# sundy-li/strawboat

Measured on AMD Instinct MI355X. Metric: encode+decode GB/s (uncompressed Arrow bytes) per GPU; 1/2/4/8-GPU scaling, higher is better.
Workload: dtype f64 bit patterns (integer/bit work, no arithmetic); 1 GPU; C2: 512 x 1M-row nullable Float64 columns per GPU, 64Ki-row pages, codec adaptive, inputs resident in HBM; columns_per_gpu=512, rows_per_column=1000000, page_rows=65536, parallelism=pages of independent columns sharded across 1 GPU(s)

## Files before the change

strawboat_amd/csrc/sb_aggregate.h:

```cpp
#pragma once

namespace sb {

struct AggAcc {
    uint64_t cnt = 0, nans = 0, kmin = ~0ull, kmax = 0, s0 = 0, s1 = 0;
};
__device__ __forceinline__ bool agg_is_float(uint32_t kind) { return kind == FK_F32 || kind == FK_F64; }
__device__ __forceinline__ double agg_dbl(uint64_t b) { return __longlong_as_double((long long)b); }
__device__ __forceinline__ uint64_t agg_bits(double v) { return (uint64_t)__double_as_longlong(v); }
__device__ __forceinline__ uint64_t agg_sext(uint64_t raw, uint32_t w) {
    const uint32_t sh = 64 - 8 * w;
    return (uint64_t)((int64_t)(raw << sh) >> sh);
}
__device__ __forceinline__ uint64_t agg_key(uint32_t kind, uint32_t w, uint64_t raw) {
    if (kind == FK_UNSIGNED) return raw;
    if (kind == FK_SIGNED) return agg_sext(raw, w) ^ (1ull << 63);
    if (kind == FK_F32) {
        const uint32_t b = (uint32_t)raw;
        return (b >> 31) ? (uint32_t)~b : (b | 0x80000000u);
    }
    return (raw >> 63) ? ~raw : (raw | (1ull << 63));
}
__device__ __forceinline__ uint64_t agg_unkey(uint32_t kind, uint32_t w, uint64_t key) {
    if (kind == FK_UNSIGNED) return key;
// ... 198 lines not shown
            agg_span(k, acc, kind, w, lo, hi, [&](uint64_t r) { return (uint64_t)s_a[sidx((int)(r - lo))]; });
            break;
        }
        default:
            return;
    }
    acc = agg_wg_reduce(acc, agg_is_float(kind), s_red);
    if (threadIdx.x == 0) agg_store(al.parts + al.tile_base + t.first_tile + tt.tile, acc);
}

__global__ void __launch_bounds__(WG) k_agg(DecodeArgs a, AggLaunch al) {
    __shared__ uint32_t s_a[SIDX_WORDS];
    __shared__ uint32_t s_w[4];
    __shared__ uint64_t s_red[AGG_RED_WORDS];
    const uint32_t count = a.job_counts[2];
    for (uint32_t ti = blockIdx.x; ti < count; ti += gridDim.x) {
        agg_tile(a, al, ti, s_a, s_w, s_red);
        __syncthreads();
    }
}

struct RleAggregate {
    using Rec = uint64_t;
    uint64_t* s_rec;
    AggSink k;
    AggAcc* acc;
    uint32_t kind, w;
    __device__ __forceinline__ uint32_t rec_bytes() const { return 4 + w; }
    __device__ __forceinline__ uint64_t load(const uint8_t* v, bool in) const { return in ? flt_load(v, w) : 0ull; }
    __device__ __forceinline__ void rows(uint64_t tile_lo, uint64_t lo, uint64_t hi, uint32_t A, const uint32_t* s_flag) const {
        agg_span(k, *acc, kind, w, lo, hi, [&](uint64_t r) { return s_rec[A + s_flag[sidx((int)(r - tile_lo))]]; });
    }
};

__global__ void __launch_bounds__(WG) k_agg_rle(DecodeArgs a, AggLaunch al) {
    __shared__ __attribute__((aligned(16))) uint32_t s_flag[SIDX_WORDS];
    __shared__ uint64_t s_vals[RLE_CHUNK];
    __shared__ uint32_t s_w[4];
    __shared__ uint64_t s_w64[4];
    __shared__ uint64_t s_red[AGG_RED_WORDS];
    if (a.job_counts[4] == 0) return;
    const uint32_t p = blockIdx.x;
    const PageDesc d = a.descs[p];
    const PageTask t = a.tasks[p];
    const ColDesc c = a.cols[t.col];
    if (!rle_by_page(c, d)) return;
// ... 148 lines not shown
```

strawboat_amd/csrc/sb_aggregate_grouped.h:

```cpp
#pragma once

namespace sb {

typedef __attribute__((address_space(3))) uint64_t* l64p;
constexpr uint32_t GF_SEL = 0, GF_CNT = 1, GF_NANS = 2, GF_KMIN = 3, GF_KMAX = 4, GF_SUM = 5;
constexpr uint32_t GRP_TREE_IDS = 4;
constexpr uint32_t GRP_LDS_WORDS =(GF_SUM + WG / 64) * GRP_MAX_GROUPS;
template <uint32_t S = GRP_MAX_GROUPS>
__device__ __forceinline__ uint64_t* grp_field(uint64_t* s_g, uint32_t f) { return s_g + f * S; }
__device__ __forceinline__ void grp_lds_add(uint64_t* p, uint64_t v) {
    (void)__hip_atomic_fetch_add((l64p)p, v, __ATOMIC_RELAXED, __HIP_MEMORY_SCOPE_WORKGROUP);
}

struct GrpSink {
    const uint32_t* sel;
    const uint8_t* def_bits;
    uint64_t out_row;
    const uint8_t* ids;
    uint32_t idw, G;
    uint64_t* s_g;
    bool all_null;
};
__device__ __forceinline__ uint32_t grp_id(const uint8_t* ids, uint32_t w, uint64_t c) {
    return w == 1 ? (uint32_t)ldu8(ids + c) : w == 2 ? (uint32_t)ldu16(ids + 2 * c) : ldu32(ids + 4 * c);
// ... 199 lines not shown
    }
    if (!agg_any_selected(g.sel, t.out_row + lo, t.out_row + hi)) return;
    grp_table_clear(s_g, gc.n_groups);
    const GrpSink k{g.sel, d.def_bits, t.out_row, gc.ids, gc.idw, gc.n_groups, s_g, false};
    uint64_t oor = 0;
    if (!grp_tile_rows(a, d, t, c, k, oor, kind, tt.page, tt.tile, lo, hi, s_a, s_w)) return;
    grp_store(gl, tt.col, gl.tile_base + t.first_tile + tt.tile, gc.n_groups, agg_is_float(kind), s_g, oor, s_w64);
}

__global__ void __launch_bounds__(WG) k_grp(DecodeArgs a, GrpLaunch gl) {
    __shared__ uint32_t s_a[SIDX_WORDS];
    __shared__ uint32_t s_w[4];
    __shared__ uint64_t s_w64[4];
    __shared__ uint64_t s_g[GRP_LDS_WORDS];
    const uint32_t count = a.job_counts[2];
    for (uint32_t ti = blockIdx.x; ti < count; ti += gridDim.x) {
        grp_tile(a, gl, ti, s_a, s_w, s_g, s_w64);
        __syncthreads();
    }
}

struct RleGrouped {
    using Rec = uint64_t;
    uint64_t* s_rec;
    GrpSink k;
    uint64_t* oor;
    uint32_t kind, w;
    __device__ __forceinline__ uint32_t rec_bytes() const { return 4 + w; }
    __device__ __forceinline__ uint64_t load(const uint8_t* v, bool in) const { return in ? flt_load(v, w) : 0ull; }
    __device__ __forceinline__ void rows(uint64_t tile_lo, uint64_t lo, uint64_t hi, uint32_t A, const uint32_t* s_flag) const {
        grp_span<true>(k, *oor, kind, w, lo, hi, [&](uint64_t r, uint64_t& raw) { return raw = s_rec[A + s_flag[sidx((int)(r - tile_lo))]], true; });
    }
};

__global__ void __launch_bounds__(WG) k_grp_rle(DecodeArgs a, GrpLaunch gl) {
    __shared__ __attribute__((aligned(16))) uint32_t s_flag[SIDX_WORDS];
    __shared__ uint64_t s_vals[RLE_CHUNK];
    __shared__ uint32_t s_w[4];
    __shared__ uint64_t s_w64[4];
    __shared__ uint64_t s_g[GRP_LDS_WORDS];
    if (a.job_counts[4] == 0) return;
    const uint32_t p = blockIdx.x;
    const PageDesc d = a.descs[p];
    const PageTask t = a.tasks[p];
    const ColDesc c = a.cols[t.col];
    if (!rle_by_page(c, d)) return;
// ... 161 lines not shown
```

strawboat_amd/csrc/sb_aggregate_grouped_large.h:

```cpp
#pragma once

namespace sb {

constexpr uint32_t GRPL_LDS_WORDS = (GF_SUM + WG / 64) * GRPL_MAX_GROUPS;
constexpr uint32_t GRPL_FINISH_GROUPS = 256;

__device__ __forceinline__ bool grpl_tile(const DecodeArgs& a, const GrpLaunch& gl, uint32_t col, const ColDesc& c, const AggCol& g, const GrpCol& gc,
                                          uint32_t page, uint32_t tile, bool& live, uint64_t& oor, uint32_t* s_a, uint32_t* s_w, uint64_t* s_g) {
    const PageDesc d = a.descs[page];
    if (!d.ok) return false;
    const PageTask t = a.tasks[page];
    const uint64_t lo = (uint64_t)tile * TILE_ROWS;
    if (lo >= t.num_values) return false;
    const uint64_t hi = min(t.num_values, lo + TILE_ROWS);
    if (d.codec == SB_CODEC_FREQ) {
        if (threadIdx.x == 0 && tile == 0) {
            gst64(gl.flags + gl.slots + gl.n_cols + col, 1);
            if (gl.replayed) raise(a.status, SB_ERR_NYI, page, 411);
            else atomicOr(&a.status->kinds, KIND_REPLAY | KIND_FILTER_FREQ);
        }
        return false;
    }
    if (rle_by_page(c, d)) return false;
    if (!agg_any_selected(g.sel, t.out_row + lo, t.out_row + hi)) return false;
// ... 23 lines not shown
    const AggCol g = gl.acols[col];
    if (slot < g.tile_slot0 || slot - g.tile_slot0 >= g.tile_slots) return;
    if (!(g.ops & AGG_VALUE_OPS)) return;
    const ColDesc c = a.cols[col];
    if (!c.n_pages) return;
    const GrpCol gc = gl.gcols[col];
    const PageTask last = a.tasks[c.first_page + c.n_pages - 1];
    const uint64_t t0 = a.tasks[c.first_page].first_tile;
    const uint64_t t1 = (uint64_t)last.first_tile + (last.num_values + TILE_ROWS - 1) / TILE_ROWS;
    const uint64_t j0 = (slot - g.tile_slot0) * GRPL_CHUNK_TILES;
    const uint64_t j1 = min(t1 - t0, j0 + GRPL_CHUNK_TILES);
    bool live = false;
    uint64_t oor = 0;
    for (uint64_t j = j0; j < j1; j++) {
        const uint32_t gt = (uint32_t)(t0 + j);
        const uint32_t page = grpl_page_of(a.tasks, c.first_page, c.n_pages, gt);
        (void)grpl_tile(a, gl, col, c, g, gc, page, gt - a.tasks[page].first_tile, live, oor, s_a, s_w, s_g);
    }
    if (live) grp_store<GRPL_MAX_GROUPS>(gl, col, slot, gc.n_groups, agg_is_float(g.kind), s_g, oor, s_w64);
}

struct RleGroupedLarge {
    using Rec = uint64_t;
    uint64_t* s_rec;
    GrpSink k;
    uint64_t* oor;
    uint32_t kind, w;
    __device__ __forceinline__ uint32_t rec_bytes() const { return 4 + w; }
    __device__ __forceinline__ uint64_t load(const uint8_t* v, bool in) const { return in ? flt_load(v, w) : 0ull; }
    __device__ __forceinline__ void rows(uint64_t tile_lo, uint64_t lo, uint64_t hi, uint32_t A, const uint32_t* s_flag) const {
        grp_span<true, GRPL_MAX_GROUPS>(k, *oor, kind, w, lo, hi,
                                        [&](uint64_t r, uint64_t& raw) { return raw = s_rec[A + s_flag[sidx((int)(r - tile_lo))]], true; });
    }
};

__global__ void __launch_bounds__(WG) k_grpl_rle(DecodeArgs a, GrpLaunch gl) {
    __shared__ __attribute__((aligned(16))) uint32_t s_flag[SIDX_WORDS];
    __shared__ uint64_t s_vals[RLE_CHUNK];
    __shared__ uint32_t s_w[4];
    __shared__ uint64_t s_w64[4];
    __shared__ uint64_t s_g[GRPL_LDS_WORDS];
    if (a.job_counts[4] == 0) return;
    const uint32_t p = blockIdx.x;
    const PageDesc d = a.descs[p];
    const PageTask t = a.tasks[p];
    const ColDesc c = a.cols[t.col];
// ... 175 lines not shown
```

strawboat_amd/csrc/sb_aggregate_weighted.h:

```cpp
#pragma once

namespace sb {

constexpr uint32_t WF_SEL = 0, WF_CNT = 1, WF_NANS = 2, WF_SUM = 3;
constexpr uint32_t WGT_FIELDS = WF_SUM + WG / 64;
constexpr uint32_t WGT_LDS_WORDS = WGT_FIELDS * GRPL_MAX_GROUPS;

__device__ __forceinline__ uint64_t* wgt_field(uint64_t* s_g, uint32_t f) { return s_g + f * GRPL_MAX_GROUPS; }

__device__ __forceinline__ void wgt_table_clear(uint64_t* s_g, uint32_t G) {
    for (uint32_t i = threadIdx.x; i < G; i += WG) {
#pragma unroll
        for (uint32_t f = 0; f < WGT_FIELDS; f++) wgt_field(s_g, f)[i] = 0ull;
    }
    __syncthreads();
}

__device__ __forceinline__ uint64_t wgt_ext(uint32_t kind, uint32_t w, uint64_t raw) { return kind == FK_SIGNED ? agg_sext(raw, w) : raw; }
__device__ __forceinline__ double wgt_dbl(uint32_t kind, uint32_t w, uint64_t raw) {
    return kind == FK_F32 ? (double)__uint_as_float((uint32_t)raw) : kind == FK_F64 ? agg_dbl(raw) : kind == FK_SIGNED ? (double)(int64_t)agg_sext(raw, w) : (double)raw;
}

template <bool VAL, class V>
__device__ __forceinline__ void wgt_span(const GrpSink& k, const WgtCol& wc, uint64_t& oor, uint32_t kind, uint32_t w, uint64_t lo, uint64_t hi, V value_of) {
// ... 201 lines not shown
    if (slot < g.tile_slot0 || slot - g.tile_slot0 >= g.tile_slots) return;
    if (!(g.ops & AGG_VALUE_OPS)) return;
    const ColDesc c = a.cols[col];
    if (!c.n_pages) return;
    const GrpCol gc = gl.gcols[col];
    const WgtCol wc = wl.wcols[col];
    const PageTask last = a.tasks[c.first_page + c.n_pages - 1];
    const uint64_t t0 = a.tasks[c.first_page].first_tile;
    const uint64_t t1 = (uint64_t)last.first_tile + (last.num_values + TILE_ROWS - 1) / TILE_ROWS;
    const uint64_t j0 = (slot - g.tile_slot0) * GRPL_CHUNK_TILES;
    const uint64_t j1 = min(t1 - t0, j0 + GRPL_CHUNK_TILES);
    bool live = false;
    uint64_t oor = 0;
    for (uint64_t j = j0; j < j1; j++) {
        const uint32_t gt = (uint32_t)(t0 + j);
        const uint32_t page = grpl_page_of(a.tasks, c.first_page, c.n_pages, gt);
        wgt_tile(a, gl, col, c, g, gc, wc, page, gt - a.tasks[page].first_tile, live, oor, s_a, s_w, s_g);
    }
    if (live) wgt_store(gl, col, slot, gc.n_groups, wc.flt, s_g, oor, s_w64);
}

struct RleWeighted {
    using Rec = uint64_t;
    uint64_t* s_rec;
    GrpSink k;
    WgtCol wc;
    uint64_t* oor;
    uint32_t kind, w;
    __device__ __forceinline__ uint32_t rec_bytes() const { return 4 + w; }
    __device__ __forceinline__ uint64_t load(const uint8_t* v, bool in) const { return in ? flt_load(v, w) : 0ull; }
    __device__ __forceinline__ void rows(uint64_t tile_lo, uint64_t lo, uint64_t hi, uint32_t A, const uint32_t* s_flag) const {
        wgt_span<true>(k, wc, *oor, kind, w, lo, hi, [&](uint64_t r, uint64_t& raw) { return raw = s_rec[A + s_flag[sidx((int)(r - tile_lo))]], true; });
    }
};

__global__ void __launch_bounds__(WG) k_wgt_rle(DecodeArgs a, WgtLaunch wl) {
    __shared__ __attribute__((aligned(16))) uint32_t s_flag[SIDX_WORDS];
    __shared__ uint64_t s_vals[RLE_CHUNK];
    __shared__ uint32_t s_w[4];
    __shared__ uint64_t s_w64[4];
    __shared__ uint64_t s_g[WGT_LDS_WORDS];
    if (a.job_counts[4] == 0) return;
    const GrpLaunch& gl = wl.gl;
    const uint32_t p = blockIdx.x;
    const PageDesc d = a.descs[p];
    const PageTask t = a.tasks[p];
// ... 184 lines not shown
```

strawboat_amd/csrc/sb_decode.hip:

```cpp
#include "sb_host.h"
#include "sb_zstd.h"
#include "sb_zstd_blocks.h"
#include "sb_lz4.h"
#include "sb_lz4_big.h"
#include "sb_lz4_giant.h"

namespace sb {

__device__ __forceinline__ bool is_basic(uint32_t c) { return c <= 3; }
__device__ __forceinline__ bool is_binary(int32_t t) { return t == SB_TYPE_BINARY || t == SB_TYPE_LARGE_BINARY; }
__device__ __forceinline__ uint32_t ballot_half(uint64_t m) { return (threadIdx.x & 32) ? (uint32_t)(m >> 32) : (uint32_t)m; }

__device__ __forceinline__ void push_job(InflateJob* q, uint32_t* cnt, const uint8_t* src, uint32_t csize,
                                         uint8_t* dst, uint32_t out_len, uint32_t codec, uint32_t page);
__device__ __forceinline__ void push_job_if(bool pred, InflateJob* q, uint32_t* cnt, const uint8_t* src, uint32_t csize, uint8_t* dst,
                                            uint32_t out_len, uint32_t codec, uint32_t page) {
    const uint64_t m = __ballot(pred);
    if (!m) return;
    const uint32_t rank = __builtin_amdgcn_mbcnt_hi((uint32_t)(m >> 32), __builtin_amdgcn_mbcnt_lo((uint32_t)m, 0));
    uint32_t base = 0;
    if (pred && rank == 0) base = __hip_atomic_fetch_add(cnt, (uint32_t)__popcll(m), __ATOMIC_RELAXED, __HIP_MEMORY_SCOPE_AGENT);
    base = (uint32_t)__builtin_amdgcn_readlane((int)base, __builtin_ctzll(m));
    if (pred) {
        InflateJob j;
// ... 2482 lines not shown
                              const uint64_t* sums ) {
    const uint32_t REC = p.rec_bytes();
    const int tid = threadIdx.x;
    const uint64_t N = t.num_values;
    const uint8_t* body = d.body;
    const uint8_t* page_end = c.pages + t.in_off + t.length;
    const uint32_t max_runs = (uint32_t)((uint64_t)(page_end - body) / REC);
    uint32_t ncnt[RLE_RPT];
    typename P::Rec nrec[RLE_RPT];
    auto fetch = [&](uint32_t base) {
#pragma unroll
        for (int j = 0; j < RLE_RPT; j++) {
            const uint32_t k = base + (uint32_t)tid * RLE_RPT + j;
            const bool in = k < max_runs;
            const uint8_t* r = body + (uint64_t)(in ? k : 0) * REC;
            ncnt[j] = in ? ldu32(r) : 0;
            nrec[j] = p.load(r + 4, in);
        }
    };
    const RlePart pt = rle_part(max_runs, part, parts);
    if (pt.none) return;
    uint64_t carry = 0;
    for (uint32_t q = 0; q < part; q++) carry += sums[q];
    if (max_runs) fetch(pt.b0);
    for (uint64_t base64 = pt.b0; carry < N && base64 < pt.b1; base64 += RLE_CHUNK) {
        const uint32_t base = (uint32_t)base64;
        if (base64 >= max_runs) {
            if (tid == 0) raise(st, SB_ERR_IO, page, 200);
            return;
        }
        uint32_t cnt[RLE_RPT];
#pragma unroll
        for (int j = 0; j < RLE_RPT; j++) {
            cnt[j] = ncnt[j];
            p.s_rec[tid * RLE_RPT + j] = nrec[j];
        }
        if (base + RLE_CHUNK < max_runs) fetch(base + RLE_CHUNK);
        uint64_t loc[RLE_RPT], run = 0;
#pragma unroll
        for (int j = 0; j < RLE_RPT; j++) {
            run += cnt[j];
            loc[j] = run;
        }
        const uint64_t incl = wave_incl_scan64(run);
        __syncthreads();
        if ((tid & 63) == 63) s_w64[tid >> 6] = incl;
        __syncthreads();
        uint64_t pre = carry + incl - run;
        const int w = tid >> 6;
        if (w > 0) pre += s_w64[0];
        if (w > 1) pre += s_w64[1];
        if (w > 2) pre += s_w64[2];
        const uint64_t chunk_total = s_w64[0] + s_w64[1] + s_w64[2] + s_w64[3];
        uint64_t start[RLE_RPT];
#pragma unroll
        for (int j = 0; j < RLE_RPT; j++) start[j] = pre + (j ? loc[j - 1] : 0);
        const uint64_t S0 = carry, S1 = min(N, carry + chunk_total);
#pragma unroll
        for (int j = 0; j < RLE_RPT; j++)
            if (start[j] < N && start[j] + cnt[j] > N) raise(st, SB_ERR_OUT_OF_SPEC, page, 202);
        for (uint64_t tile_lo = S0 / TILE_ROWS * TILE_ROWS; tile_lo < S1; tile_lo += TILE_ROWS) {
            const uint64_t lo = max(S0, tile_lo), hi = min(S1, tile_lo + TILE_ROWS);
            static_assert(SIDX_WORDS % 4 == 0, "16-byte clears");
            for (int i = tid; i < SIDX_WORDS / 4; i += WG) ((u32x4*)s_flag)[i] = u32x4{0, 0, 0, 0};
            uint32_t le = 0;
#pragma unroll
            for (int j = 0; j < RLE_RPT; j++) le += (base + (uint32_t)tid * RLE_RPT + j < max_runs && start[j] <= lo) ? 1u : 0u;
            __syncthreads();
#pragma unroll
            for (int j = 0; j < RLE_RPT; j++)
                if (base + (uint32_t)tid * RLE_RPT + j < max_runs && start[j] > lo && start[j] < hi)
                    atomicAdd(&s_flag[sidx((int)(start[j] - tile_lo))], 1u);
            uint32_t v = le;
#pragma unroll
            for (int dlt = 32; dlt > 0; dlt >>= 1) v += __shfl_down(v, dlt, 64);
            if ((tid & 63) == 0) s_w[tid >> 6] = v;
            __syncthreads();
            const uint32_t A = s_w[0] + s_w[1] + s_w[2] + s_w[3] - 1;
            __syncthreads();
            tile_incl_scan(s_flag, s_w);
            p.rows(tile_lo, lo, hi, A, s_flag);
            __syncthreads();
        }
        carry += chunk_total;
        if (chunk_total == 0 && base + RLE_CHUNK >= max_runs && carry < N) {
            if (tid == 0) raise(st, SB_ERR_IO, page, 200);
            return;
        }
    }
}

template <int W>
struct RleExpand {
    using Rec = Val<W>;
    Val<W>* s_rec;
    uint8_t* dst;
    __device__ __forceinline__ uint32_t rec_bytes() const { return 4 + W; }
    __device__ __forceinline__ Val<W> load(const uint8_t* v, bool in) const { return in ? ld_val<W>(v) : Val<W>{}; }
    __device__ __forceinline__ void rows(uint64_t tile_lo, uint64_t lo, uint64_t hi, uint32_t A, const uint32_t* s_flag) const {
        const uint32_t off = (uint32_t)(lo - tile_lo);
        emit_rows<W>(dst + lo * W, (uint32_t)(hi - lo), [&](uint32_t i) { return s_rec[A + s_flag[sidx((int)(off + i))]]; });
    }
};
template <int W>
__device__ __forceinline__ void expand_rle_page(const ColDesc& c, const PageTask& t, const PageDesc& d, uint32_t* s_flag, uint8_t* s_vals,
                                                uint32_t* s_w, uint64_t* s_w64, Status* st, uint32_t page, uint32_t part, uint32_t parts,
                                                const uint64_t* sums) {
    rle_page_walk(RleExpand<W>{(Val<W>*)s_vals, c.values + t.out_row * W}, c, t, d, s_flag, s_w, s_w64, st, page, part, parts, sums);
}

__device__ void page_copy_bits(uint8_t* dst_bm, uint64_t dst_bit0, const uint8_t* src, uint64_t N, bool aligned) {
    constexpr int U = 8;
    const uint32_t nwords = (uint32_t)((N + 31) / 32);
    for (uint32_t g0 = threadIdx.x; g0 < nwords; g0 += WG * U) {
        uint32_t v[U];
#pragma unroll
        for (int u = 0; u < U; u++) {
// ... 386 lines not shown
```

strawboat_amd/csrc/sb_filter.h:

```cpp
#pragma once

namespace sb {

constexpr uint32_t FILTER_DICT_BITS = 8192;

struct FilterCmp {
    uint64_t lit;
    uint32_t kind, mask, w;
};
__device__ __forceinline__ FilterCmp filter_cmp(const FilterCol& f, uint32_t w) { return FilterCmp{f.lit, f.kind, f.mask, w}; }
__device__ __forceinline__ uint64_t flt_load(const uint8_t* p, uint32_t w) {
    switch (w) {
        case 1:
            return ldu8(p);
        case 2:
            return ldu16(p);
        case 4:
            return ldu32(p);
        default:
            return ldu64(p);
    }
}
__device__ __forceinline__ bool flt_eval(const FilterCmp& k, uint64_t raw) {
    uint32_t rel;
// ... 141 lines not shown
            U32Stream vs{d.body, (const uint32_t*)(a.scratch + t.aux_off), d.codec, 0, t.num_values};
            u32_tile_to_lds(vs, tt.tile, rows, s_a, s_w);
            filter_span(k, lo, hi, [&](uint64_t r) { return flt_eval(cmp, s_a[sidx((int)(r - lo))]); });
            break;
        }
        default:
            break;
    }
}

__global__ void __launch_bounds__(WG) k_filter(DecodeArgs a, const FilterCol* fcols) {
    __shared__ uint32_t s_a[SIDX_WORDS];
    __shared__ uint32_t s_w[4];
    __shared__ uint32_t s_tab[FILTER_DICT_BITS / 32];
    const uint32_t count = a.job_counts[2];
    for (uint32_t ti = blockIdx.x; ti < count; ti += gridDim.x) {
        filter_tile(a, fcols, ti, s_a, s_w, s_tab);
        __syncthreads();
    }
}

struct RleFilter {
    using Rec = uint8_t;
    uint8_t* s_rec;
    FilterSink k;
    FilterCmp cmp;
    __device__ __forceinline__ uint32_t rec_bytes() const { return 4 + cmp.w; }
    __device__ __forceinline__ uint8_t load(const uint8_t* v, bool in) const { return in && flt_eval(cmp, flt_load(v, cmp.w)); }
    __device__ __forceinline__ void rows(uint64_t tile_lo, uint64_t lo, uint64_t hi, uint32_t A, const uint32_t* s_flag) const {
        filter_span(k, lo, hi, [&](uint64_t r) { return s_rec[A + s_flag[sidx((int)(r - tile_lo))]] != 0; });
    }
};

__global__ void __launch_bounds__(WG) k_filter_rle(DecodeArgs a, const FilterCol* fcols) {
    __shared__ __attribute__((aligned(16))) uint32_t s_flag[SIDX_WORDS];
    __shared__ uint8_t s_pred[RLE_CHUNK];
    __shared__ uint32_t s_w[4];
    __shared__ uint64_t s_w64[4];
    if (a.job_counts[4] == 0) return;
    const uint32_t p = blockIdx.x;
    const PageDesc d = a.descs[p];
    const PageTask t = a.tasks[p];
    const ColDesc c = a.cols[t.col];
    if (!rle_by_page(c, d)) return;
    const FilterCol f = fcols[t.col];
    if (f.op >= SB_PRED_IS_NULL) return;
// ... 108 lines not shown
```

strawboat_amd/csrc/sb_filter_in.h:

```cpp
#pragma once

namespace sb {

struct InEval {
    const uint64_t* keys;
    uint32_t n, steps, negate, kind, w;
};
__device__ __forceinline__ bool in_member(const uint64_t* keys, uint32_t n, uint32_t steps, uint64_t x) {
    uint32_t pos = 0;
    for (uint32_t s = steps; s-- > 0;) {
        const uint32_t p = pos + (1u << s);
        const uint64_t k = keys[min(p, n) - 1];
        pos = (p <= n && k < x) ? p : pos;
    }
    return n != 0 && pos < n && keys[min(pos, n - 1)] == x;
}
__device__ __forceinline__ bool in_eval(const InEval& k, uint64_t raw) {
    return in_member(k.keys, k.n, k.steps, in_key(k.kind, k.w, raw)) != (k.negate != 0);
}
__device__ __forceinline__ void in_stage(const InCol& ic, uint64_t* s_keys) {
    const uint32_t n = min(ic.n, IN_MAX_VALUES);
    for (uint32_t i = threadIdx.x; i < n; i += WG) s_keys[i] = ic.keys[i];
}
__device__ __forceinline__ InEval in_eval_of(const FilterCol& f, const InCol& ic, const uint64_t* s_keys, uint32_t w) {
// ... 71 lines not shown
            filter_span(k, lo, hi, [&](uint64_t r) { return in_eval(ev, s_a[sidx((int)(r - lo))]); });
            break;
        }
        default:
            break;
    }
}

__global__ void __launch_bounds__(WG) k_filter_in(DecodeArgs a, const FilterCol* fcols, const InCol* icols) {
    __shared__ uint32_t s_a[SIDX_WORDS];
    __shared__ uint32_t s_w[4];
    __shared__ uint32_t s_tab[FILTER_DICT_BITS / 32];
    __shared__ uint64_t s_keys[IN_MAX_VALUES];
    const uint32_t count = a.job_counts[2];
    uint32_t staged = 0xFFFFFFFFu;
    for (uint32_t ti = blockIdx.x; ti < count; ti += gridDim.x) {
        filter_in_tile(a, fcols, icols, ti, s_a, s_w, s_tab, s_keys, &staged);
        __syncthreads();
    }
}

struct RleFilterIn {
    using Rec = uint8_t;
    uint8_t* s_rec;
    FilterSink k;
    InEval ev;
    __device__ __forceinline__ uint32_t rec_bytes() const { return 4 + ev.w; }
    __device__ __forceinline__ uint8_t load(const uint8_t* v, bool in) const { return in && in_eval(ev, flt_load(v, ev.w)); }
    __device__ __forceinline__ void rows(uint64_t tile_lo, uint64_t lo, uint64_t hi, uint32_t A, const uint32_t* s_flag) const {
        filter_span(k, lo, hi, [&](uint64_t r) { return s_rec[A + s_flag[sidx((int)(r - tile_lo))]] != 0; });
    }
};

__global__ void __launch_bounds__(WG) k_filter_in_rle(DecodeArgs a, const FilterCol* fcols, const InCol* icols) {
    __shared__ __attribute__((aligned(16))) uint32_t s_flag[SIDX_WORDS];
    __shared__ uint8_t s_pred[RLE_CHUNK];
    __shared__ uint32_t s_w[4];
    __shared__ uint64_t s_w64[4];
    __shared__ uint64_t s_keys[IN_MAX_VALUES];
    if (a.job_counts[4] == 0) return;
    const uint32_t p = blockIdx.x;
    const PageDesc d = a.descs[p];
    const PageTask t = a.tasks[p];
    const ColDesc c = a.cols[t.col];
    if (!rle_by_page(c, d)) return;
    const FilterCol f = fcols[t.col];
// ... 173 lines not shown
```

strawboat_amd/csrc/sb_key_buckets.h:

```cpp
#pragma once

namespace sb {

constexpr uint32_t BUCK_NAN = 0xFFFFu;
constexpr uint32_t BUCK_BAD = 0xFFFEu;
static_assert(BUCK_MAX_BOUNDS + 1 <= KEY_MAX_KEYS && BUCK_MAX_BOUNDS < BUCK_BAD, "a bucket code fits 16 bits beside the markers");

struct BuckFind {
    const uint64_t* keys;
    const uint32_t* bid;
    uint64_t nan_lo, nan_hi;
    uint32_t n, steps, kind, w, rc, nan_id;
};
template <bool FLT>
__device__ __forceinline__ uint32_t buck_code(const BuckFind& f, uint64_t raw) {
    const uint64_t x = in_key(f.kind, f.w, raw);
    uint32_t pos = key_lower_bound(f.keys, f.n, f.steps, x);
    if (!f.rc && pos < f.n && f.keys[pos] == x) pos++;
    if (FLT && (x < f.nan_lo || x > f.nan_hi)) pos = BUCK_NAN;
    return pos;
}
__device__ __forceinline__ uint32_t buck_id(const BuckFind& f, uint32_t code) {
    return code <= f.n ? f.bid[code] : code == BUCK_NAN ? f.nan_id : LOOK_NONE;
}
// ... 155 lines not shown
    if (flt) key_buckets_rows<true>(a, tt, d, t, c, b, f, lo, rows, s_a, s_w, s_pos);
    else key_buckets_rows<false>(a, tt, d, t, c, b, f, lo, rows, s_a, s_w, s_pos);
    buck_store(b, flt, bl.st + tt.col, s_cnt);
}

__global__ void __launch_bounds__(WG) k_key_buckets(DecodeArgs a, BuckLaunch bl) {
    __shared__ uint32_t s_a[SIDX_WORDS];
    __shared__ uint32_t s_w[4];
    __shared__ unsigned long long s_cnt[3];
    __shared__ uint16_t s_pos[FILTER_DICT_BITS];
    __shared__ uint64_t s_keys[KEY_MAX_KEYS];
    __shared__ uint32_t s_bid[KEY_MAX_KEYS];
    const uint32_t count = a.job_counts[2];
    uint32_t staged = 0xFFFFFFFFu;
    for (uint32_t ti = blockIdx.x; ti < count; ti += gridDim.x) {
        key_buckets_tile(a, bl, ti, s_a, s_w, s_pos, s_keys, s_bid, s_cnt, &staged);
        __syncthreads();
    }
}

template <bool FLT>
struct RleKeyBuckets {
    using Rec = uint32_t;
    uint32_t* s_rec;
    BuckSink* b;
    BuckFind f;
    __device__ __forceinline__ uint32_t rec_bytes() const { return 4 + f.w; }
    __device__ __forceinline__ uint32_t load(const uint8_t* v, bool in) const {
        if (!in) return FLT ? BUCK_BAD : LOOK_NONE;
        const uint32_t code = buck_code<FLT>(f, flt_load(v, f.w));
        return FLT ? code : buck_id(f, code);
    }
    __device__ __forceinline__ void rows(uint64_t tile_lo, uint64_t lo, uint64_t hi, uint32_t A, const uint32_t* s_flag) const {
        if (FLT) buck_span_f(*b, f, lo, hi, [&](uint64_t r) { return s_rec[A + s_flag[sidx((int)(r - tile_lo))]]; });
        else look_span(b->k, lo, hi, [&](uint64_t r) { return s_rec[A + s_flag[sidx((int)(r - tile_lo))]]; });
    }
};

__global__ void __launch_bounds__(WG) k_key_buckets_rle(DecodeArgs a, BuckLaunch bl) {
    __shared__ __attribute__((aligned(16))) uint32_t s_flag[SIDX_WORDS];
    __shared__ uint32_t s_run[RLE_CHUNK];
    __shared__ uint32_t s_w[4];
    __shared__ uint64_t s_w64[4];
    __shared__ unsigned long long s_cnt[3];
    __shared__ uint64_t s_keys[KEY_MAX_KEYS];
    __shared__ uint32_t s_bid[KEY_MAX_KEYS];
// ... 99 lines not shown
```

strawboat_amd/csrc/sb_key_ids.h:

```cpp
#pragma once

namespace sb {

constexpr uint32_t KEY_SET_SLOTS = 2048;
static_assert(KEY_SET_SLOTS >= KEY_MAX_KEYS + 2 * WG && (KEY_SET_SLOTS & (KEY_SET_SLOTS - 1)) == 0, "never full; a power of two");

__device__ __forceinline__ uint32_t key_hash(uint64_t key) { return (uint32_t)((key * 0x9E3779B97F4A7C15ull) >> 40); }
__device__ __forceinline__ uint32_t key_over(const KeyState* st) {
    return __hip_atomic_load(&st->overflow, __ATOMIC_RELAXED, __HIP_MEMORY_SCOPE_AGENT);
}

struct KeySink {
    const uint32_t* sel;
    const uint8_t* def_bits;
    uint64_t out_row;
    uint64_t* set;
    KeyState* st;
    uint64_t* tab;
    uint32_t mask, max_keys;
    uint64_t cnt = 0;
    uint32_t zero = 0;
};
__device__ __forceinline__ KeySink key_sink(const KeyLaunch& kl, uint32_t col, uint64_t* set, const uint32_t* sel, const uint8_t* def_bits, uint64_t out_row) {
    const KeyCol kc = kl.kcols[col];
// ... 158 lines not shown
        }
        default:
            return;
    }
    key_store(s, s_w64);
}

__global__ void __launch_bounds__(WG) k_key_collect(DecodeArgs a, KeyLaunch kl) {
    __shared__ uint32_t s_a[SIDX_WORDS];
    __shared__ uint32_t s_w[4];
    __shared__ uint64_t s_w64[4];
    __shared__ uint32_t s_tab[FILTER_DICT_BITS / 32];
    __shared__ uint64_t s_set[KEY_SET_SLOTS];
    const uint32_t count = a.job_counts[2];
    uint32_t owner = 0xFFFFFFFFu;
    for (uint32_t ti = blockIdx.x; ti < count; ti += gridDim.x) {
        key_collect_tile(a, kl, ti, s_a, s_w, s_tab, s_set, s_w64, &owner);
        __syncthreads();
    }
}

struct RleKeyCollect {
    using Rec = uint64_t;
    uint64_t* s_rec;
    KeySink* k;
    uint32_t kind, w;
    __device__ __forceinline__ uint32_t rec_bytes() const { return 4 + w; }
    __device__ __forceinline__ uint64_t load(const uint8_t* v, bool in) const { return in ? in_key(kind, w, flt_load(v, w)) : 0ull; }
    __device__ __forceinline__ void rows(uint64_t tile_lo, uint64_t lo, uint64_t hi, uint32_t A, const uint32_t* s_flag) const {
        key_span(*k, lo, hi, [&](uint64_t r) { return s_rec[A + s_flag[sidx((int)(r - tile_lo))]]; });
    }
};

__global__ void __launch_bounds__(WG) k_key_collect_rle(DecodeArgs a, KeyLaunch kl) {
    __shared__ __attribute__((aligned(16))) uint32_t s_flag[SIDX_WORDS];
    __shared__ uint64_t s_vals[RLE_CHUNK];
    __shared__ uint32_t s_w[4];
    __shared__ uint64_t s_w64[4];
    __shared__ uint64_t s_set[KEY_SET_SLOTS];
    if (a.job_counts[4] == 0) return;
    const uint32_t p = blockIdx.x;
    const PageDesc d = a.descs[p];
    const PageTask t = a.tasks[p];
    const ColDesc c = a.cols[t.col];
    if (!rle_by_page(c, d)) return;
    const AggCol g = kl.acols[t.col];
// ... 193 lines not shown
            key_id_span(k, lo, hi, [&](uint64_t r) { return key_find(f, (uint64_t)s_a[sidx((int)(r - lo))]); });
            break;
        }
        default:
            break;
    }
}

__global__ void __launch_bounds__(WG) k_key_assign(DecodeArgs a, KeyLaunch kl) {
    __shared__ uint32_t s_a[SIDX_WORDS];
    __shared__ uint32_t s_w[4];
    __shared__ uint16_t s_ids[FILTER_DICT_BITS];
    __shared__ uint64_t s_keys[KEY_MAX_KEYS];
    const uint32_t count = a.job_counts[2];
    uint32_t staged = 0xFFFFFFFFu;
    for (uint32_t ti = blockIdx.x; ti < count; ti += gridDim.x) {
        key_assign_tile(a, kl, ti, s_a, s_w, s_ids, s_keys, &staged);
        __syncthreads();
    }
}

struct RleKeyAssign {
    using Rec = uint32_t;
    uint32_t* s_rec;
    KeyIdSink k;
    KeyFind f;
    __device__ __forceinline__ uint32_t rec_bytes() const { return 4 + f.w; }
    __device__ __forceinline__ uint32_t load(const uint8_t* v, bool in) const { return in ? key_find(f, flt_load(v, f.w)) : 0u; }
    __device__ __forceinline__ void rows(uint64_t tile_lo, uint64_t lo, uint64_t hi, uint32_t A, const uint32_t* s_flag) const {
        key_id_span(k, lo, hi, [&](uint64_t r) { return s_rec[A + s_flag[sidx((int)(r - tile_lo))]]; });
    }
};

__global__ void __launch_bounds__(WG) k_key_assign_rle(DecodeArgs a, KeyLaunch kl) {
    __shared__ __attribute__((aligned(16))) uint32_t s_flag[SIDX_WORDS];
    __shared__ uint32_t s_run[RLE_CHUNK];
    __shared__ uint32_t s_w[4];
    __shared__ uint64_t s_w64[4];
    __shared__ uint64_t s_keys[KEY_MAX_KEYS];
    if (a.job_counts[4] == 0) return;
    const uint32_t p = blockIdx.x;
    const PageDesc d = a.descs[p];
    const PageTask t = a.tasks[p];
    const ColDesc c = a.cols[t.col];
    if (!rle_by_page(c, d)) return;
    if (kl.st[t.col].overflow) return;
// ... 71 lines not shown
```

strawboat_amd/csrc/sb_key_lookup.h:

```cpp
#pragma once

namespace sb {

constexpr uint32_t LOOK_NONE = 0xFFFFFFFFu;
constexpr uint32_t LOOK_NOPOS = 0xFFFFu;
static_assert(KEY_MAX_KEYS <= LOOK_NOPOS, "a sorted position fits 16 bits beside the marker");

struct LookSink {
    const uint32_t* sel;
    const uint8_t* def_bits;
    uint64_t out_row;
    uint8_t* ids;
    uint32_t idw;
    uint32_t live = 0, hit = 0;
};
template <class F>
__device__ __forceinline__ void look_span(LookSink& k, uint64_t lo, uint64_t hi, F id_of) {
    for (uint64_t base = lo; base < hi; base += WG) {
        const uint64_t r = base + threadIdx.x, c = k.out_row + r;
        const bool in = r < hi;
        bool on = in;
        if (on && k.sel) on = (gld32(k.sel + (c >> 5)) >> (uint32_t)(c & 31)) & 1u;
        if (on && k.def_bits) on = (ldu8(k.def_bits + (r >> 3)) >> (uint32_t)(r & 7)) & 1u;
        const uint32_t id = on ? id_of(r) : LOOK_NONE;
// ... 125 lines not shown
        default:
            return;
    }
    look_store(k, ll.st + tt.col, s_cnt);
}

__global__ void __launch_bounds__(WG) k_key_lookup(DecodeArgs a, LookLaunch ll) {
    __shared__ uint32_t s_a[SIDX_WORDS];
    __shared__ uint32_t s_w[4];
    __shared__ unsigned long long s_cnt[2];
    __shared__ uint16_t s_pos[FILTER_DICT_BITS];
    __shared__ uint64_t s_keys[KEY_MAX_KEYS];
    __shared__ uint32_t s_kid[KEY_MAX_KEYS];
    const uint32_t count = a.job_counts[2];
    uint32_t staged = 0xFFFFFFFFu;
    for (uint32_t ti = blockIdx.x; ti < count; ti += gridDim.x) {
        key_lookup_tile(a, ll, ti, s_a, s_w, s_pos, s_keys, s_kid, s_cnt, &staged);
        __syncthreads();
    }
}

struct RleKeyLookup {
    using Rec = uint32_t;
    uint32_t* s_rec;
    LookSink* k;
    LookFind f;
    __device__ __forceinline__ uint32_t rec_bytes() const { return 4 + f.w; }
    __device__ __forceinline__ uint32_t load(const uint8_t* v, bool in) const { return in ? look_find(f, flt_load(v, f.w)) : LOOK_NONE; }
    __device__ __forceinline__ void rows(uint64_t tile_lo, uint64_t lo, uint64_t hi, uint32_t A, const uint32_t* s_flag) const {
        look_span(*k, lo, hi, [&](uint64_t r) { return s_rec[A + s_flag[sidx((int)(r - tile_lo))]]; });
    }
};

__global__ void __launch_bounds__(WG) k_key_lookup_rle(DecodeArgs a, LookLaunch ll) {
    __shared__ __attribute__((aligned(16))) uint32_t s_flag[SIDX_WORDS];
    __shared__ uint32_t s_run[RLE_CHUNK];
    __shared__ uint32_t s_w[4];
    __shared__ uint64_t s_w64[4];
    __shared__ unsigned long long s_cnt[2];
    __shared__ uint64_t s_keys[KEY_MAX_KEYS];
    __shared__ uint32_t s_kid[KEY_MAX_KEYS];
    if (a.job_counts[4] == 0) return;
    const uint32_t p = blockIdx.x;
    const PageDesc d = a.descs[p];
    const PageTask t = a.tasks[p];
    const ColDesc c = a.cols[t.col];
// ... 208 lines not shown
```

strawboat_amd/csrc/sb_read_sel.h:

```cpp
#pragma once

namespace sb {

__device__ __forceinline__ uint64_t sel_rank_at(const SelCol& s, uint64_t c) {
    const uint64_t g = c >> 5;
    const uint32_t b = (uint32_t)(c & 31);
    uint64_t r = gld64(s.rank + g);
    if (b) r += (uint64_t)__popc(gld32(s.sel + g) & ((1u << b) - 1));
    return r;
}

__device__ __forceinline__ void sel_store(uint8_t* p, uint64_t v, uint32_t w) {
    switch (w) {
        case 1:
            *(gptr)p = (uint8_t)v;
            break;
        case 2: {
            const uint16_t x = (uint16_t)v;
            __builtin_memcpy((gptr)p, &x, 2);
            break;
        }
        case 4:
            stu32(p, (uint32_t)v);
            break;
// ... 125 lines not shown
            U32Stream vs{d.body, (const uint32_t*)(a.scratch + t.aux_off), d.codec, 0, t.num_values};
            u32_tile_to_lds(vs, tt.tile, rows, s_a, s_w);
            sel_span(k, lo, hi, [&](uint64_t r) { return (uint64_t)s_a[sidx((int)(r - lo))]; });
            break;
        }
        default:
            break;
    }
}

__global__ void __launch_bounds__(WG) k_rsel(DecodeArgs a, const SelCol* scols) {
    __shared__ uint32_t s_a[SIDX_WORDS];
    __shared__ uint32_t s_w[4];
    __shared__ uint32_t s_strip[WG];
    const uint32_t count = a.job_counts[2];
    for (uint32_t ti = blockIdx.x; ti < count; ti += gridDim.x) {
        rsel_tile(a, scols, ti, s_a, s_w, s_strip);
        __syncthreads();
    }
}

struct RleSelect {
    using Rec = uint64_t;
    uint64_t* s_rec;
    SelSink k;
    __device__ __forceinline__ uint32_t rec_bytes() const { return 4 + k.s.w; }
    __device__ __forceinline__ uint64_t load(const uint8_t* v, bool in) const { return in ? flt_load(v, k.s.w) : 0ull; }
    __device__ __forceinline__ void rows(uint64_t tile_lo, uint64_t lo, uint64_t hi, uint32_t A, const uint32_t* s_flag) const {
        if (sel_rank_at(k.s, k.out_row + lo) == sel_rank_at(k.s, k.out_row + hi)) return;
        sel_span(k, lo, hi, [&](uint64_t r) { return s_rec[A + s_flag[sidx((int)(r - tile_lo))]]; });
    }
};

__global__ void __launch_bounds__(WG) k_rsel_rle(DecodeArgs a, const SelCol* scols) {
    __shared__ __attribute__((aligned(16))) uint32_t s_flag[SIDX_WORDS];
    __shared__ uint64_t s_vals[RLE_CHUNK];
    __shared__ uint32_t s_w[4];
    __shared__ uint64_t s_w64[4];
    __shared__ uint32_t s_strip[WG];
    if (a.job_counts[4] == 0) return;
    const uint32_t p = blockIdx.x;
    const PageDesc d = a.descs[p];
    const PageTask t = a.tasks[p];
    const ColDesc c = a.cols[t.col];
    if (!rle_by_page(c, d)) return;
    const uint32_t part = blockIdx.y, parts = gridDim.y;
// ... 108 lines not shown
```

strawboat_amd/csrc/sb_topk.h:

```cpp
#pragma once

namespace sb {

constexpr uint32_t TOPK_CAP = 1024;
constexpr uint32_t TOPK_FINISH_STEPS = (TOPK_CAP - TOPK_MAX_K) / WG;
static_assert((TOPK_CAP & (TOPK_CAP - 1)) == 0 && TOPK_CAP >= TOPK_MAX_K + WG, "a power of two that holds k records and a step");
static_assert(TOPK_MAX_K <= WG, "k_topk_finish takes a slot's records in one step");

struct TopkBuf {
    uint64_t key[TOPK_CAP], row[TOPK_CAP];
    uint64_t bkey, brow;
    uint32_t n, pad;
};

struct TopkSink {
    const uint32_t* sel;
    const uint8_t* def_bits;
    uint64_t out_row;
    TopkBuf* b;
    uint32_t k;
    uint64_t flip;
    uint64_t cnt = 0, nans = 0;
    uint64_t bkey = ~0ull, brow = ~0ull;
    uint32_t room = 1;
// ... 168 lines not shown
            topk_span(s, kind, w, lo, hi, [&](uint64_t r, uint64_t& raw) { return raw = (uint64_t)s_a[sidx((int)(r - lo))], true; });
            break;
        }
        default:
            return;
    }
    topk_store(s, tl, tl.tile_base + t.first_tile + tt.tile, s_w64);
}

__global__ void __launch_bounds__(WG) k_topk(DecodeArgs a, TopkLaunch tl) {
    __shared__ uint32_t s_a[SIDX_WORDS];
    __shared__ uint32_t s_w[4];
    __shared__ uint64_t s_w64[4];
    __shared__ TopkBuf s_t;
    const uint32_t count = a.job_counts[2];
    for (uint32_t ti = blockIdx.x; ti < count; ti += gridDim.x) {
        topk_tile(a, tl, ti, s_a, s_w, &s_t, s_w64);
        __syncthreads();
    }
}

struct RleTopk {
    using Rec = uint64_t;
    uint64_t* s_rec;
    TopkSink* k;
    uint32_t kind, w;
    __device__ __forceinline__ uint32_t rec_bytes() const { return 4 + w; }
    __device__ __forceinline__ uint64_t load(const uint8_t* v, bool in) const { return in ? flt_load(v, w) : 0ull; }
    __device__ __forceinline__ void rows(uint64_t tile_lo, uint64_t lo, uint64_t hi, uint32_t A, const uint32_t* s_flag) const {
        topk_span(*k, kind, w, lo, hi, [&](uint64_t r, uint64_t& raw) { return raw = s_rec[A + s_flag[sidx((int)(r - tile_lo))]], true; });
    }
};

__global__ void __launch_bounds__(WG) k_topk_rle(DecodeArgs a, TopkLaunch tl) {
    __shared__ __attribute__((aligned(16))) uint32_t s_flag[SIDX_WORDS];
    __shared__ uint64_t s_vals[RLE_CHUNK];
    __shared__ uint32_t s_w[4];
    __shared__ uint64_t s_w64[4];
    __shared__ TopkBuf s_t;
    if (a.job_counts[4] == 0) return;
    const uint32_t p = blockIdx.x;
    const PageDesc d = a.descs[p];
    const PageTask t = a.tasks[p];
    const ColDesc c = a.cols[t.col];
    if (!rle_by_page(c, d)) return;
    const AggCol g = tl.acols[t.col];
// ... 116 lines not shown
```

Measured before the change: 3953 GB/s.

## Align RLE expand chunks to whole tile boundaries

For the RLE expand path, each chunk of runs now ends at the last complete tile boundary. The run that straddles that boundary is refetched at the start of the next chunk, so output tiles are written whole and not split across chunk iterations. This trades one extra barrier and a search per chunk, plus re-reading some runs, for less partial-tile handling. Other RLE consumers keep the old behaviour through a compile-time flag.

```diff
diff --git a/strawboat_amd/csrc/sb_aggregate.h b/strawboat_amd/csrc/sb_aggregate.h
--- a/strawboat_amd/csrc/sb_aggregate.h
+++ b/strawboat_amd/csrc/sb_aggregate.h
@@ -244,6 +244,7 @@
 
 struct RleAggregate {
     using Rec = uint64_t;
+    static constexpr bool whole_tiles = false;
     uint64_t* s_rec;
     AggSink k;
     AggAcc* acc;
diff --git a/strawboat_amd/csrc/sb_aggregate_grouped.h b/strawboat_amd/csrc/sb_aggregate_grouped.h
--- a/strawboat_amd/csrc/sb_aggregate_grouped.h
+++ b/strawboat_amd/csrc/sb_aggregate_grouped.h
@@ -245,6 +245,7 @@
 
 struct RleGrouped {
     using Rec = uint64_t;
+    static constexpr bool whole_tiles = false;
     uint64_t* s_rec;
     GrpSink k;
     uint64_t* oor;
diff --git a/strawboat_amd/csrc/sb_aggregate_grouped_large.h b/strawboat_amd/csrc/sb_aggregate_grouped_large.h
--- a/strawboat_amd/csrc/sb_aggregate_grouped_large.h
+++ b/strawboat_amd/csrc/sb_aggregate_grouped_large.h
@@ -69,6 +69,7 @@
 
 struct RleGroupedLarge {
     using Rec = uint64_t;
+    static constexpr bool whole_tiles = false;
     uint64_t* s_rec;
     GrpSink k;
     uint64_t* oor;
diff --git a/strawboat_amd/csrc/sb_aggregate_weighted.h b/strawboat_amd/csrc/sb_aggregate_weighted.h
--- a/strawboat_amd/csrc/sb_aggregate_weighted.h
+++ b/strawboat_amd/csrc/sb_aggregate_weighted.h
@@ -247,6 +247,7 @@
 
 struct RleWeighted {
     using Rec = uint64_t;
+    static constexpr bool whole_tiles = false;
     uint64_t* s_rec;
     GrpSink k;
     WgtCol wc;
diff --git a/strawboat_amd/csrc/sb_decode.hip b/strawboat_amd/csrc/sb_decode.hip
--- a/strawboat_amd/csrc/sb_decode.hip
+++ b/strawboat_amd/csrc/sb_decode.hip
@@ -2528,8 +2528,9 @@
     if (pt.none) return;
     uint64_t carry = 0;
     for (uint32_t q = 0; q < part; q++) carry += sums[q];
+    uint64_t from = carry;
     if (max_runs) fetch(pt.b0);
-    for (uint64_t base64 = pt.b0; carry < N && base64 < pt.b1; base64 += RLE_CHUNK) {
+    for (uint64_t base64 = pt.b0; carry < N && base64 < pt.b1;) {
         const uint32_t base = (uint32_t)base64;
         if (base64 >= max_runs) {
             if (tid == 0) raise(st, SB_ERR_IO, page, 200);
@@ -2541,7 +2542,8 @@
             cnt[j] = ncnt[j];
             p.s_rec[tid * RLE_RPT + j] = nrec[j];
         }
-        if (base + RLE_CHUNK < max_runs) fetch(base + RLE_CHUNK);
+        if constexpr (!P::whole_tiles)
+            if (base + RLE_CHUNK < max_runs) fetch(base + RLE_CHUNK);
         uint64_t loc[RLE_RPT], run = 0;
 #pragma unroll
         for (int j = 0; j < RLE_RPT; j++) {
@@ -2551,6 +2553,8 @@
         const uint64_t incl = wave_incl_scan64(run);
         __syncthreads();
         if ((tid & 63) == 63) s_w64[tid >> 6] = incl;
+        if constexpr (P::whole_tiles)
+            if (tid == 0) s_w[0] = 0;
         __syncthreads();
         uint64_t pre = carry + incl - run;
         const int w = tid >> 6;
@@ -2561,7 +2565,27 @@
         uint64_t start[RLE_RPT];
 #pragma unroll
         for (int j = 0; j < RLE_RPT; j++) start[j] = pre + (j ? loc[j - 1] : 0);
-        const uint64_t S0 = carry, S1 = min(N, carry + chunk_total);
+        uint64_t S0 = carry, S1 = min(N, carry + chunk_total);
+        uint32_t step = RLE_CHUNK, back = 0;
+        if constexpr (P::whole_tiles) {
+            S0 = from;
+            const uint64_t E = S1 / TILE_ROWS * TILE_ROWS;
+            if (parts == 1 && base + RLE_CHUNK < max_runs && carry + chunk_total < N && E > from) {
+#pragma unroll
+                for (int j = 0; j < RLE_RPT; j++)
+                    if (tid * RLE_RPT + j > 0 && start[j] <= E && E - start[j] < cnt[j]) {
+                        s_w[0] = (uint32_t)tid * RLE_RPT + j;
+                        s_w[1] = (uint32_t)(E - start[j]);
+                    }
+            }
+            __syncthreads();
+            if (s_w[0]) {
+                step = s_w[0];
+                back = s_w[1];
+                S1 = E;
+            }
+            if (base + step < max_runs) fetch(base + step);
+        }
 #pragma unroll
         for (int j = 0; j < RLE_RPT; j++)
             if (start[j] < N && start[j] + cnt[j] > N) raise(st, SB_ERR_OUT_OF_SPEC, page, 202);
@@ -2588,7 +2612,13 @@
             p.rows(tile_lo, lo, hi, A, s_flag);
             __syncthreads();
         }
-        carry += chunk_total;
+        if constexpr (P::whole_tiles) {
+            from = S1;
+            carry = step == RLE_CHUNK ? carry + chunk_total : S1 - back;
+        } else {
+            carry += chunk_total;
+        }
+        base64 += step;
         if (chunk_total == 0 && base + RLE_CHUNK >= max_runs && carry < N) {
             if (tid == 0) raise(st, SB_ERR_IO, page, 200);
             return;
@@ -2596,9 +2626,13 @@
     }
 }
 
+#ifndef SB_RLE_WHOLE_TILES
+#define SB_RLE_WHOLE_TILES 1
+#endif
 template <int W>
 struct RleExpand {
     using Rec = Val<W>;
+    static constexpr bool whole_tiles = SB_RLE_WHOLE_TILES != 0;
     Val<W>* s_rec;
     uint8_t* dst;
     __device__ __forceinline__ uint32_t rec_bytes() const { return 4 + W; }
diff --git a/strawboat_amd/csrc/sb_filter.h b/strawboat_amd/csrc/sb_filter.h
--- a/strawboat_amd/csrc/sb_filter.h
+++ b/strawboat_amd/csrc/sb_filter.h
@@ -187,6 +187,7 @@
 
 struct RleFilter {
     using Rec = uint8_t;
+    static constexpr bool whole_tiles = false;
     uint8_t* s_rec;
     FilterSink k;
     FilterCmp cmp;
diff --git a/strawboat_amd/csrc/sb_filter_in.h b/strawboat_amd/csrc/sb_filter_in.h
--- a/strawboat_amd/csrc/sb_filter_in.h
+++ b/strawboat_amd/csrc/sb_filter_in.h
@@ -117,6 +117,7 @@
 
 struct RleFilterIn {
     using Rec = uint8_t;
+    static constexpr bool whole_tiles = false;
     uint8_t* s_rec;
     FilterSink k;
     InEval ev;
diff --git a/strawboat_amd/csrc/sb_key_buckets.h b/strawboat_amd/csrc/sb_key_buckets.h
--- a/strawboat_amd/csrc/sb_key_buckets.h
+++ b/strawboat_amd/csrc/sb_key_buckets.h
@@ -201,6 +201,7 @@
 template <bool FLT>
 struct RleKeyBuckets {
     using Rec = uint32_t;
+    static constexpr bool whole_tiles = false;
     uint32_t* s_rec;
     BuckSink* b;
     BuckFind f;
diff --git a/strawboat_amd/csrc/sb_key_ids.h b/strawboat_amd/csrc/sb_key_ids.h
--- a/strawboat_amd/csrc/sb_key_ids.h
+++ b/strawboat_amd/csrc/sb_key_ids.h
@@ -204,6 +204,7 @@
 
 struct RleKeyCollect {
     using Rec = uint64_t;
+    static constexpr bool whole_tiles = false;
     uint64_t* s_rec;
     KeySink* k;
     uint32_t kind, w;
@@ -443,6 +444,7 @@
 
 struct RleKeyAssign {
     using Rec = uint32_t;
+    static constexpr bool whole_tiles = false;
     uint32_t* s_rec;
     KeyIdSink k;
     KeyFind f;
diff --git a/strawboat_amd/csrc/sb_key_lookup.h b/strawboat_amd/csrc/sb_key_lookup.h
--- a/strawboat_amd/csrc/sb_key_lookup.h
+++ b/strawboat_amd/csrc/sb_key_lookup.h
@@ -171,6 +171,7 @@
 
 struct RleKeyLookup {
     using Rec = uint32_t;
+    static constexpr bool whole_tiles = false;
     uint32_t* s_rec;
     LookSink* k;
     LookFind f;
diff --git a/strawboat_amd/csrc/sb_read_sel.h b/strawboat_amd/csrc/sb_read_sel.h
--- a/strawboat_amd/csrc/sb_read_sel.h
+++ b/strawboat_amd/csrc/sb_read_sel.h
@@ -171,6 +171,7 @@
 
 struct RleSelect {
     using Rec = uint64_t;
+    static constexpr bool whole_tiles = false;
     uint64_t* s_rec;
     SelSink k;
     __device__ __forceinline__ uint32_t rec_bytes() const { return 4 + k.s.w; }
diff --git a/strawboat_amd/csrc/sb_topk.h b/strawboat_amd/csrc/sb_topk.h
--- a/strawboat_amd/csrc/sb_topk.h
+++ b/strawboat_amd/csrc/sb_topk.h
@@ -214,6 +214,7 @@
 
 struct RleTopk {
     using Rec = uint64_t;
+    static constexpr bool whole_tiles = false;
     uint64_t* s_rec;
     TopkSink* k;
     uint32_t kind, w;
```

New measurement: 3918 GB/s. Within noise of the previous version (-0.9%).
